# xdsopl/dwt

Hardware: AMD Instinct MI355X
Metric: Mpixels/s lossless encode+decode round-trip (higher is better)
Workload: dtype int32; 1 GPU; 4096x4096x1 8-bit synthetic smooth+noise frames, lossless, 128 frames per GPU per step (BASELINE.json configs[1] geometry); frames_per_gpu=128, parallelism=1 GPU

## Files before the change

dwt_amd/csrc/pack.hip:

```cpp
#include "hilbert_dev.h"

#include <stdlib.h>
#include <string.h>

namespace {

constexpr int TILE = 1024;
constexpr int NCUM = 32;
constexpr int MAX_PLANES = 16;
constexpr int MAX_SEGS = 3 * 16 * MAX_PLANES;
constexpr int SUB = 64;
constexpr int CHUNK = SUB * 64;
constexpr int GROUP = 64;

constexpr unsigned T_RUN = 0x0fffu, T_ESC = 0x0fffu, T_BREAK = 1u << 13, T_VOID = 1u << 14, T_NOSIGN = 1u << 15;

struct PackGeom {
	int levels, C, W, H;
	long total;
	const int *pyr;
	const short *fine16;
	unsigned lv16;
	unsigned sq_levels;
	int side[DWTX_MAX_LEVELS + 1];
	int pixels[DWTX_MAX_LEVELS + 1];
	int tile_first[DWTX_MAX_LEVELS + 1];
	const int *tile_base;
	const unsigned short *tile_cnt;
	const int *tile_blk;
};

struct ImgInfo {
	int planes[3];
	int pmax;
	int K;
	int E;
	unsigned T;
	int order0;
	unsigned hdr_bits;
	unsigned root_bits;
	unsigned meta_bits;
	unsigned cut;
	unsigned long long total_bits;
	unsigned long long nbytes;
	int error;
	int pad;
};

struct RunMap {
	unsigned keep, add;
};

struct Work {
	unsigned short *cum;
	unsigned *tile_mx;
	ImgInfo *info;
	int *seg_desc;
	int *seg_ebase;
	unsigned *seg_refs;
	unsigned long long *seg_rawoff;
	unsigned *brk_tok;
	int *segidx;
	unsigned *live;
	unsigned short *ent_ones, *ent_zeros, *ent_refs, *ent_tz;
	unsigned short *ent_seg;
	unsigned *ent_tokbase;
	unsigned *ent_refscum;
	unsigned *ent_refw;
	unsigned short *tok16;
	unsigned *tok_big;
	unsigned *stage;
	unsigned char *grp_ord;
	unsigned long long *lane_bits;
	unsigned char *sublut;
	unsigned char *lut;
	unsigned char *glut;
	unsigned char *chunk_entry;
	unsigned char *group_entry;
	unsigned long long *chunk_bits;
	unsigned long long *chunk_base;
	RunMap *carry_agg;
	unsigned *carry_in;
	unsigned *ent_blk;
	unsigned long long *stream_bits;
	int *slow;
	long ES, TS, NCS, NGS, NCB, SW;
	int NT, NTP;
	unsigned *seg_run;
};

__device__ __forceinline__ int lane_id()
{
	return __builtin_amdgcn_mbcnt_hi(~0u, __builtin_amdgcn_mbcnt_lo(~0u, 0));
}

__device__ __forceinline__ int popc_below(unsigned long long m)
{
	return __builtin_amdgcn_mbcnt_hi((unsigned)(m >> 32), __builtin_amdgcn_mbcnt_lo((unsigned)m, 0));
}

__device__ __forceinline__ int ilog2u(unsigned v) { return 31 - __builtin_clz(v); }

__device__ __forceinline__ void wave_sync()
{
	__builtin_amdgcn_fence(__ATOMIC_RELEASE, "wavefront");
	__builtin_amdgcn_wave_barrier();
	__builtin_amdgcn_fence(__ATOMIC_ACQUIRE, "wavefront");
}

__device__ __forceinline__ unsigned wave_incl_add(unsigned v)
{
	v += (unsigned)__builtin_amdgcn_update_dpp(0, (int)v, 0x111, 0xf, 0xf, false);
	v += (unsigned)__builtin_amdgcn_update_dpp(0, (int)v, 0x112, 0xf, 0xf, false);
	v += (unsigned)__builtin_amdgcn_update_dpp(0, (int)v, 0x114, 0xf, 0xf, false);
	v += (unsigned)__builtin_amdgcn_update_dpp(0, (int)v, 0x118, 0xf, 0xf, false);
	v += (unsigned)__builtin_amdgcn_update_dpp(0, (int)v, 0x142, 0xa, 0xf, false);
	v += (unsigned)__builtin_amdgcn_update_dpp(0, (int)v, 0x143, 0xc, 0xf, false);
	return v;
}

__device__ __forceinline__ unsigned bfm_mask(unsigned width)
{
	unsigned r;
	asm("v_bfm_b32 %0, %1, 0" : "=v"(r) : "v"(width));
	return r;
}
__device__ __forceinline__ int vli_top(int o, unsigned v) { return ilog2u(v + (1u << o)); }
__device__ __forceinline__ int vli_next(int top) { return top >= 2 ? top - 2 : 0; }

__device__ __forceinline__ void seg_unpack(int d, int &c, int &l, int &p)
{
	c = d & 15;
	l = (d >> 4) & 15;
	p = (d >> 8) - 1;
}

struct __attribute__((packed, aligned(4))) Int4U {
	int x, y, z, w;
};

__device__ __forceinline__ void load_tile16(const PackGeom &g, const int *__restrict__ lin, int plane, int l, int tile, int lane, int nvalid,
	int nv, unsigned *lds, int (&val)[16])
{
	if (((g.sq_levels >> l) & 1u) && nvalid == TILE) {
		if ((g.lv16 >> l) & 1u)
			load_square16(g.fine16 + (long)plane * g.total, g.W, g.side[l], g.tile_blk[tile], lane, lds, val);
		else
			load_square16(g.pyr + (long)plane * g.total, g.W, g.side[l], g.tile_blk[tile], lane, lds, val);
		return;
	}
	const int tbase = g.tile_base[tile];
	const int *src = lin + (long)plane * g.total + g.pixels[l] + tbase + 16 * lane;
	const int k = (int)(((uintptr_t)src >> 2) & 3);
// ... 481 lines not shown
	const unsigned tb = block_excl_scan(nt, wsum, tt);
	const unsigned rb = block_excl_scan(nr, wsum, rt);
	const unsigned wb = block_excl_scan((nr + 31u) >> 5, wsum, wt);
	if (e < E) {
		w.ent_tokbase[img * (w.ES + 1) + e] = tb;
		w.ent_refscum[img * (w.ES + 1) + e] = rb;
		w.ent_refw[img * (w.ES + 1) + e] = wb;
	}
	if (threadIdx.x == 0) {
		w.ent_blk[(img * w.NCB + blockIdx.x) * 3] = tt;
		w.ent_blk[(img * w.NCB + blockIdx.x) * 3 + 1] = rt;
		w.ent_blk[(img * w.NCB + blockIdx.x) * 3 + 2] = wt;
	}
}

__global__ __launch_bounds__(ENT_BLOCK) void k_entries_blocks(Work w)
{
	__shared__ unsigned wsum[16];
	const int img = blockIdx.x;
	ImgInfo &I = w.info[img];
	const int E = I.E;
	const int nb = (E + ENT_BLOCK - 1) / ENT_BLOCK;
	unsigned tok_run = 0, ref_run = 0, word_run = 0;
	for (int b0 = 0; b0 < nb; b0 += ENT_BLOCK) {
		const int b = b0 + threadIdx.x;
		unsigned *slot = w.ent_blk + (img * w.NCB + b) * 3;
		const unsigned t = b < nb ? slot[0] : 0u, r = b < nb ? slot[1] : 0u, wd = b < nb ? slot[2] : 0u;
		unsigned tt, rt, wt;
		const unsigned tb = block_excl_scan(t, wsum, tt);
		const unsigned rb = block_excl_scan(r, wsum, rt);
		const unsigned wb = block_excl_scan(wd, wsum, wt);
		if (b < nb) {
			slot[0] = tok_run + tb;
			slot[1] = ref_run + rb;
			slot[2] = word_run + wb;
		}
		tok_run += tt;
		ref_run += rt;
		word_run += wt;
	}
	if (threadIdx.x == 0) {
		w.ent_tokbase[img * (w.ES + 1) + E] = tok_run;
		w.ent_refscum[img * (w.ES + 1) + E] = ref_run;
		w.ent_refw[img * (w.ES + 1) + E] = word_run;
		I.T = tok_run + 1;
	}
}

__global__ __launch_bounds__(ENT_BLOCK) void k_entries_finish(Work w)
{
	const int img = blockIdx.y;
	const int e = blockIdx.x * ENT_BLOCK + threadIdx.x;
	if (e >= w.info[img].E)
		return;
	const unsigned *slot = w.ent_blk + (img * w.NCB + blockIdx.x) * 3;
	w.ent_tokbase[img * (w.ES + 1) + e] += slot[0];
	w.ent_refscum[img * (w.ES + 1) + e] += slot[1];
	w.ent_refw[img * (w.ES + 1) + e] += slot[2];
}

__global__ __launch_bounds__(ENT_BLOCK) void k_entries_segs(Work w)
{
	const int img = blockIdx.x;
	const int K = w.info[img].K;
	const int *eb = w.seg_ebase + (long)img * (MAX_SEGS + 1);
	const unsigned *tokbase = w.ent_tokbase + img * (w.ES + 1), *refscum = w.ent_refscum + img * (w.ES + 1);
	static_assert(MAX_SEGS <= ENT_BLOCK, "one thread per segment");
	const int k = threadIdx.x;
	if (k < K) {
		const unsigned refs = refscum[eb[k + 1]] - refscum[eb[k]];
		w.seg_refs[(long)img * MAX_SEGS + k] = refs;
		const int last = eb[k + 1] - 1;
		w.brk_tok[(long)img * MAX_SEGS + k] = tokbase[last] + w.ent_ones[img * w.ES + last];
	}
}

__global__ __launch_bounds__(ENT_BLOCK) void k_cut(Work w, long capacity, int cut_off)
{
	__shared__ unsigned long long need[MAX_SEGS];
	__shared__ int kc_sh;
	const int img = blockIdx.x;
	ImgInfo &I = w.info[img];
	const int K = I.K;
	const int *eb = w.seg_ebase + (long)img * (MAX_SEGS + 1);
	const unsigned *tokbase = w.ent_tokbase + img * (w.ES + 1);
	const int k = threadIdx.x;
	if (k < K) {
		const unsigned ones = tokbase[eb[k + 1]] - tokbase[eb[k]] - 1u;
		need[k] = 2ull * ones + w.seg_refs[(long)img * MAX_SEGS + k];
	}
	__syncthreads();
	if (threadIdx.x == 0) {
		int kc = K;
		if (capacity > 0 && !cut_off) {
			const unsigned long long limit = 8ull * ((unsigned long long)capacity + 1ull);
			unsigned long long at = I.hdr_bits;
			for (int j = 0; j < K; ++j) {
				if (at >= limit) {
					kc = j;
					break;
				}
				at += need[j];
			}
		}
		kc_sh = kc;
		I.cut = (unsigned)(K - kc);
		I.K = kc;
		I.E = eb[kc];
		I.T = tokbase[eb[kc]] + 1u;
	}
	__syncthreads();
	const int kc = kc_sh;
	if (threadIdx.x < 48) {
		const int *sx = w.segidx + ((long)img * 48 + threadIdx.x) * MAX_PLANES;
		unsigned m = 0;
		for (int p = 0; p < MAX_PLANES; ++p)
			m |= (sx[p] && sx[p] <= kc ? 1u : 0u) << p;
		w.live[(long)img * 48 + threadIdx.x] = m;
	}
}


__device__ __forceinline__ int tab8(int lane, int cls) { return cls * 128 + lane * 2; }
__device__ __forceinline__ int tab16(int lane, int cls) { return cls * 64 + lane; }
constexpr int ROWW = 34;
constexpr int ZS_DUMMY = TILE + 8 * MAX_PLANES, ZS_SLOTS = ZS_DUMMY + 8;

struct alignas(16) CodeLds {
	unsigned tab[1024];
	union {
		unsigned short zs[ZS_SLOTS];
		unsigned rows[(MAX_PLANES - 1) * ROWW];
	};
	unsigned short cum[MAX_PLANES + 2];
	unsigned short slot0[MAX_PLANES];
	unsigned gb[MAX_PLANES];
	unsigned long long rb[MAX_PLANES];
	int ent[MAX_PLANES];
};

template <int NQ>
struct Nib;
template <>
struct Nib<8> {
	typedef unsigned T;
	static constexpr T ONES = 0x11111111u, M0F = 0x0f0f0f0fu;
};
template <>
struct Nib<16> {
	typedef unsigned long long T;
	static constexpr T ONES = 0x1111111111111111ull, M0F = 0x0f0f0f0f0f0f0f0full;
};

__device__ __forceinline__ void transpose8(unsigned &lo, unsigned &hi)
{
	unsigned t;
	t = (lo ^ (lo >> 7)) & 0x00AA00AAu;
	lo ^= t ^ (t << 7);
	t = (hi ^ (hi >> 7)) & 0x00AA00AAu;
	hi ^= t ^ (t << 7);
	t = (lo ^ (lo >> 14)) & 0x0000CCCCu;
	lo ^= t ^ (t << 14);
	t = (hi ^ (hi >> 14)) & 0x0000CCCCu;
	hi ^= t ^ (t << 14);
	const unsigned nlo = (lo & 0x0F0F0F0Fu) | ((hi << 4) & 0xF0F0F0F0u);
	hi = ((lo >> 4) & 0x0F0F0F0Fu) | (hi & 0xF0F0F0F0u);
	lo = nlo;
}

__device__ __forceinline__ unsigned pext4_entry(unsigned i)
{
	const unsigned m = i >> 4, v = i & 15u;
	unsigned out = 0, k = 0;
#pragma unroll
	for (int j = 0; j < 4; ++j) {
		out |= (((v & m) >> j) & 1u) << k;
		k += (m >> j) & 1u;
	}
	return out;
}

typedef unsigned short ushort2_t __attribute__((ext_vector_type(2)));

__device__ __forceinline__ unsigned slots_to_tokens(unsigned a, unsigned before)
{
	const unsigned b = __builtin_amdgcn_alignbit(a, before, 16);
	const ushort2_t d = __builtin_bit_cast(ushort2_t, a & 0x03ff03ffu) - __builtin_bit_cast(ushort2_t, b & 0x03ff03ffu);
	return (a & 0x10001000u) | __builtin_bit_cast(unsigned, d);
}

template <int NQ, bool FULL>
__device__ __forceinline__ void code_tile(CodeLds &L, const unsigned char *pext4, const int (&val)[16], const Work &w, int img, int lane, int nvalid,
	int nv, int vb, int Pc, int tile_top, unsigned my_tokbase, int my_ent, unsigned long long my_rb)
{
	const int P = Pc < tile_top ? Pc : tile_top;
	typedef typename Nib<NQ>::T R_t;
	constexpr R_t ONES = Nib<NQ>::ONES, M0F = Nib<NQ>::M0F;
	constexpr int NB = NQ / 4;

	unsigned mag[16];
	unsigned sgn = 0;
	R_t Ra = 0, Rb = 0;
#pragma unroll
	for (int i = 0; i < 16; ++i) {
		const int v = val[i];
		const unsigned a = (unsigned)(v < 0 ? -v : v);
		mag[i] = a;
		sgn |= ((unsigned)v >> 31) << i;
		int t = 32 - __clz((int)a);
		t = t < NQ ? t : NQ;
		const int te = FULL || i < nv ? t : NQ;
		const R_t m = te < NQ ? ONES << (4 * te) : (R_t)0;
		if (i < 8)
			Ra += m;
		else
			Rb += m;
	}
	const R_t ev = (Ra & M0F) + (Rb & M0F);
	const R_t od = ((Ra >> 4) & M0F) + ((Rb >> 4) & M0F);
	unsigned E[NB], O[NB], cE[NB], cO[NB];
	const int nq = (P >> 2) + 1 < NB ? (P >> 2) + 1 : NB;
#pragma unroll
	for (int b = 0; b < NB; ++b) {
		const unsigned xe = (unsigned)(ev >> (16 * b)) & 0xffffu, xo = (unsigned)(od >> (16 * b)) & 0xffffu;
		const unsigned e0 = (xe & 0xffu) | ((xe & 0xff00u) << 8), o0 = (xo & 0xffu) | ((xo & 0xff00u) << 8);
		unsigned ei = 0, oi = 0;
		if (b < nq) {
			ei = wave_incl_add(e0);
			oi = wave_incl_add(o0);
		}
		cE[b] = (unsigned)__builtin_amdgcn_readlane((int)ei, 63);
		cO[b] = (unsigned)__builtin_amdgcn_readlane((int)oi, 63);
		E[b] = ei - e0;
		O[b] = oi - o0;
	}
#define ZL(q) ((((q) & 1 ? O[((q) >> 2) % NB] : E[((q) >> 2) % NB]) >> (16 * (((q) >> 1) & 1))) & 0xffffu)
#define CT(q) ((((q) & 1 ? cO[((q) >> 2) % NB] : cE[((q) >> 2) % NB]) >> (16 * (((q) >> 1) & 1))) & 0xffffu)
	unsigned first[NQ];
	{
		unsigned cur = 0;
#pragma unroll
		for (int p = NQ - 1; p >= 0; --p) {
			const unsigned c1 = p + 1 < P && p + 1 < NQ ? CT(p + 1) : (unsigned)nvalid, c0 = p < P ? CT(p) : (unsigned)nvalid;
			const unsigned tb = (unsigned)__builtin_amdgcn_readlane((int)my_tokbase, p);
			first[p] = cur + ((tb - cur) & 7u);
			cur = first[p] + (c1 - c0);
		}
	}
#pragma unroll
	for (int t = 1; t <= NQ; ++t) {
		if (t <= P) {
			const unsigned zlo = ZL(t - 1);
			const unsigned zhi = t < NQ && t < P ? ZL(t) : (unsigned)vb;
			if (NQ == 8)
				*reinterpret_cast<uint2 *>(&L.tab[tab8(lane, t - 1)]) = make_uint2(zlo, first[t - 1] + zhi - zlo);
			else
				L.tab[tab16(lane, t - 1)] = zlo | (zhi - zlo) << 10 | first[t - 1] << 20;
		}
	}
	if (lane == 0) {
#pragma unroll
		for (int q = 0; q <= MAX_PLANES; ++q)
			L.cum[q] = (unsigned short)(q < P && q < NQ ? CT(q) : (unsigned)nvalid);
#pragma unroll
		for (int q = 0; q < MAX_PLANES; ++q)
			L.slot0[q] = (unsigned short)(q < NQ ? first[q < NQ ? q : 0] : 0u);
	}
	wave_sync();

	if (lane < MAX_PLANES) {
		L.gb[lane] = my_ent >= 0 ? my_tokbase : ~0u;
		L.ent[lane] = my_ent;
		L.rb[lane] = my_rb;
	}
	wave_sync();

	auto cq = [&](int q) -> unsigned { return q < P && q < NQ ? CT(q) : (unsigned)nvalid; };

	wave_sync();
	for (int i = lane; i < (NQ - 1) * ROWW; i += 64)
		L.rows[i] = 0u;
	wave_sync();
	auto deposit = [&](int p, unsigned acc, unsigned cnt, unsigned zl, unsigned bit0) {
		const unsigned pos = (bit0 & 31u) + ((unsigned)vb - zl);
		if (cnt) {
			unsigned *row = L.rows + p * ROWW;
			const unsigned sh = pos & 31u;
			atomicOr(&row[pos >> 5], acc << sh);
			if (sh + cnt > 32u)
				atomicOr(&row[(pos >> 5) + 1], acc >> (32u - sh));
		}
	};
	unsigned *stage = w.stage + img * w.SW;
	auto row_out = [&](int p, int refs, unsigned long long bit0) {
		const int nw = (refs + 31) >> 5;
		if (lane < nw)
			stage[(bit0 >> 5) + lane] = L.rows[p * ROWW + lane];
	};
	if (NQ == 8) {
		unsigned A0 = mag[0] | mag[1] << 8 | mag[2] << 16 | mag[3] << 24, A1 = mag[4] | mag[5] << 8 | mag[6] << 16 | mag[7] << 24;
		unsigned B0 = mag[8] | mag[9] << 8 | mag[10] << 16 | mag[11] << 24, B1 = mag[12] | mag[13] << 8 | mag[14] << 16 | mag[15] << 24;
		transpose8(A0, A1);
		transpose8(B0, B1);
		const unsigned SA1 = (A1 >> 8) | (A1 >> 16) | (A1 >> 24), SB1 = (B1 >> 8) | (B1 >> 16) | (B1 >> 24);
		const unsigned SA0 = (A0 >> 8) | (A0 >> 16) | (A0 >> 24) | ((SA1 | A1) & 0xffu) * 0x01010101u;
		const unsigned SB0 = (B0 >> 8) | (B0 >> 16) | (B0 >> 24) | ((SB1 | B1) & 0xffu) * 0x01010101u;
		auto plane_string = [&](int p, unsigned Aw, unsigned SAw, unsigned Bw, unsigned SBw) {
			const int refs = nvalid - (int)L.cum[p + 1];
			if (refs <= 0 || L.ent[p] < 0)
				return;
			const unsigned sh8 = 8u * ((unsigned)p & 3u);
			const unsigned nA = (Aw >> sh8) & 0xffu, sA = (SAw >> sh8) & 0xffu, nB = (Bw >> sh8) & 0xffu, sB = (SBw >> sh8) & 0xffu;
			const unsigned e0 = pext4[((sA & 15u) << 4) | (nA & 15u)], e1 = pext4[(sA & 0xf0u) | (nA >> 4)];
			const unsigned e2 = pext4[((sB & 15u) << 4) | (nB & 15u)], e3 = pext4[(sB & 0xf0u) | (nB >> 4)];
			const unsigned c0 = (unsigned)__builtin_popcount(sA & 15u), c1 = (unsigned)__builtin_popcount(sA);
			const unsigned c2 = c1 + (unsigned)__builtin_popcount(sB & 15u), c3 = c1 + (unsigned)__builtin_popcount(sB);
			deposit(p, e0 | e1 << c0 | e2 << c1 | e3 << c2, c3, L.tab[tab8(lane, p + 1)] & 0x3ffu, (unsigned)L.rb[p]);
		};
		for (int p = P - 2; p >= 4; --p)
			plane_string(p, A1, SA1, B1, SB1);
		for (int p = P - 2 < 3 ? P - 2 : 3; p >= 0; --p)
			plane_string(p, A0, SA0, B0, SB0);
		wave_sync();
		for (int p = P - 2; p >= 0; --p) {
			const int refs = nvalid - (int)L.cum[p + 1];
			if (refs <= 0 || L.ent[p] < 0)
				continue;
			row_out(p, refs, L.rb[p]);
		}
	} else {
		for (int p = P - 2; p >= 0; --p) {
			const int refs = nvalid - (int)L.cum[p + 1];
			if (refs <= 0 || L.ent[p] < 0)
				continue;
			const unsigned thr = 2u << p;
			unsigned acc = 0, cnt = 0;
#pragma unroll
			for (int i = 0; i < 16; ++i) {
				const bool isref = mag[i] >= thr;
				acc |= (isref ? (mag[i] >> p) & 1u : 0u) << cnt;
				cnt += isref ? 1u : 0u;
			}
			deposit(p, acc, cnt, L.tab[tab16(lane, p + 1)] & 0x3ffu, (unsigned)L.rb[p]);
		}
		wave_sync();
		for (int p = P - 2; p >= 0; --p) {
			const int refs = nvalid - (int)L.cum[p + 1];
			if (refs <= 0 || L.ent[p] < 0)
				continue;
			row_out(p, refs, L.rb[p]);
		}
	}
	wave_sync();
	{
		R_t R = 0;
		constexpr int NB8 = NQ == 8 ? 8 : 2;
#pragma unroll
		for (int h = 0; h < 16 / NB8; ++h) {
			uint2 ent[NB8];
#pragma unroll
			for (int i = NB8 * h; i < NB8 * h + NB8; ++i) {
				const int t0 = min(32 - __clz((int)mag[i]), NQ);
				const int tm = t0 > 0 ? t0 - 1 : 0;
				if (NQ == 8) {
					ent[i % NB8] = *reinterpret_cast<const uint2 *>(&L.tab[tab8(lane, tm)]);
				} else {
					const unsigned e = L.tab[tab16(lane, tm)];
					ent[i % NB8] = make_uint2(e & 0x3ffu, (e >> 20) + ((e >> 10) & 0x3ffu));
				}
			}
#pragma unroll
			for (int i = NB8 * h; i < NB8 * h + NB8; ++i) {
				const int t = min(32 - __clz((int)mag[i]), NQ);
				const int tm = t > 0 ? t - 1 : 0;
				const unsigned x = (unsigned)(R >> (4 * tm));
				const unsigned lz_lo = x & 15u;
				const unsigned lz_hi = t < NQ ? (x >> 4) & 15u : (unsigned)i;
				const unsigned slot = mag[i] ? ent[i % NB8].y + lz_hi - lz_lo : (unsigned)(ZS_DUMMY + (lane & 7));
				L.zs[slot] = (unsigned short)(ent[i % NB8].x + lz_lo + ((sgn >> i) & 1u) * 0x1000u);
				const int te = FULL || i < nv ? t : NQ;
				R += te < NQ ? ONES << (4 * te) : (R_t)0;
			}
		}
	}
	wave_sync();
	{
		unsigned first_tok = 0;
		int first_slot = -1;
		if (lane < MAX_PLANES) {
			const int p = lane;
			const unsigned c0 = L.cum[p], c1 = L.cum[p + 1];
			const unsigned ones = c1 - c0, slot0 = L.slot0[p];
			if (ones) {
				first_slot = (int)slot0;
				first_tok = L.zs[slot0];
			}
			if (my_ent >= 0)
				w.ent_tz[img * w.ES + my_ent] = (unsigned short)(ones ? c0 - (L.zs[slot0 + ones - 1] & 0x3ffu) : c0);
		}
		const int nslots = (int)(first[0] + (cq(1) - cq(0)));
		uint4 *zq = reinterpret_cast<uint4 *>(L.zs);
		const int nblk = (nslots + 511) >> 9;
		unsigned before[3];
#pragma unroll
		for (int k = 0; k < 3; ++k)
			before[k] = k < nblk && 512 * k + 8 * lane > 0 && 512 * k + 8 * lane <= ZS_DUMMY ? (unsigned)L.zs[512 * k + 8 * lane - 1] << 16 : 0u;
		wave_sync();
#pragma unroll
		for (int k = 0; k < 3; ++k)
			if (k < nblk && 64 * k + lane < ZS_DUMMY / 8) {
				const uint4 a = zq[64 * k + lane];
				zq[64 * k + lane] = make_uint4(slots_to_tokens(a.x, before[k]), slots_to_tokens(a.y, a.x), slots_to_tokens(a.z, a.y), slots_to_tokens(a.w, a.z));
			}
		wave_sync();
		if (first_slot >= 0)
			L.zs[first_slot] = (unsigned short)first_tok;
		wave_sync();
		unsigned short *tok16 = w.tok16 + img * w.TS;
		auto plane_out = [&](unsigned tb, unsigned slot0, int ones) {
			unsigned short *dst = tok16 + tb;
			const unsigned short *src = L.zs + slot0;
			const int head = min(ones, (int)((8u - (tb & 7u)) & 7u));
			const int chunks = (ones - head) >> 3, tail0 = head + 8 * chunks;
			const int e = lane < 8 ? lane : tail0 + lane - 8;
			if (lane < 8 ? lane < head : (lane < 16 && e < ones))
				dst[e] = src[e];
			for (int c = lane; c < chunks; c += 64)
				*reinterpret_cast<uint4 *>(dst + head + 8 * c) = *reinterpret_cast<const uint4 *>(src + head + 8 * c);
		};
		for (int p = P > 0 ? P - 1 : 0; p >= 0; --p) {
			const unsigned c0 = (unsigned)__builtin_amdgcn_readfirstlane((int)L.cum[p]), c1 = (unsigned)__builtin_amdgcn_readfirstlane((int)L.cum[p + 1]);
			const int ones = (int)(c1 - c0);
			const unsigned gb = (unsigned)__builtin_amdgcn_readfirstlane((int)L.gb[p]);
			if (ones <= 0 || gb == ~0u)
				continue;
			plane_out(gb, (unsigned)__builtin_amdgcn_readfirstlane((int)L.slot0[p]), ones);
		}
	}

#undef ZL
#undef CT
}

template <bool WIDE>
__device__ __forceinline__ void code_one(const PackGeom &g, const int *__restrict__ lin, const Work &w, CodeLds &L, const unsigned char *pext4, int tile,
	int plane, int lane)
{
	const int img = plane / g.C, c = plane - img * g.C;
	const ImgInfo &I = w.info[img];
	{
	int l = 0;
	while (l + 1 < g.levels && tile >= g.tile_first[l + 1])
		++l;
	const int j = tile - g.tile_first[l];
	const int nvalid = g.tile_cnt[tile];
	const int P = I.planes[c] < MAX_PLANES ? I.planes[c] : MAX_PLANES;
	const unsigned live = w.live[(long)img * 48 + c * 16 + l];
	if (!live)
		return;
	const unsigned tile_or = w.tile_mx[(long)plane * w.NTP + tile];
	const int tile_top = tile_or ? ilog2u(tile_or) + 1 : 0;
	if (!(live & ((1u << (tile_top < 31 ? tile_top : 31)) - 1u))) {
		if (lane < MAX_PLANES && ((live >> lane) & 1u)) {
			const int k = w.segidx[((long)img * 48 + c * 16 + l) * MAX_PLANES + lane] - 1;
			w.ent_tz[img * w.ES + w.seg_ebase[(long)img * (MAX_SEGS + 1) + k] + j] = (unsigned short)nvalid;
		}
		return;
	}
	const int first = 16 * lane;
	const int nv = nvalid - first < 0 ? 0 : nvalid - first > 16 ? 16 : nvalid - first;
	const int vb = first < nvalid ? first : nvalid;

	static_assert(sizeof(L.tab) >= sizeof(unsigned) * SQ_WORDS, "the class table doubles as the square's staging area");
	int val[16];
	load_tile16(g, lin, plane, l, tile, lane, nvalid, nv, L.tab, val);
// ... 442 lines not shown
		const unsigned xs[2] = { x2.x, x2.y };
#pragma unroll
		for (int h = 0; h < 2; ++h) {
			const unsigned x = xs[h];
			if (pair_is_special(x)) {
				const unsigned v[2] = { token_run(x & 0xffffu, big, tb + 4 * q + 2 * h), token_run(x >> 16, big, tb + 4 * q + 2 * h + 1) };
				pair_bits(x, v, tb + 4 * q + 2 * h, lo, count_raw, btok, srefs, K, tokbits, rawbits);
			} else {
				pair_bits_plain(x, tb + 4 * q + 2 * h, lo, count_raw, btok, srefs, K, tokbits, rawbits);
			}
		}
	}
	if (met)
		hi = lo;
	return qmet;
}

__device__ __forceinline__ void walk_bits(const unsigned *my, const unsigned *big, long tb, int o, int qend, bool count_raw,
	const unsigned *btok, const unsigned *srefs, int K, unsigned &tokbits, unsigned long long &rawbits)
{
#pragma unroll 2
	for (int q = 0; q < qend; ++q) {
		const uint2 x2 = *reinterpret_cast<const uint2 *>(my + 2 * q);
		const unsigned xs[2] = { x2.x, x2.y };
#pragma unroll
		for (int h = 0; h < 2; ++h) {
			const unsigned x = xs[h];
			if (pair_is_special(x)) {
				const unsigned v[2] = { token_run(x & 0xffffu, big, tb + 4 * q + 2 * h), token_run(x >> 16, big, tb + 4 * q + 2 * h + 1) };
				pair_bits(x, v, tb + 4 * q + 2 * h, o, count_raw, btok, srefs, K, tokbits, rawbits);
			} else {
				pair_bits_plain(x, tb + 4 * q + 2 * h, o, count_raw, btok, srefs, K, tokbits, rawbits);
			}
		}
	}
}

constexpr int FSUBS = 63;

struct WalkLds {
	unsigned tok[64 * WROW];
};

constexpr int GO_WAVES = 2;

__global__ __launch_bounds__(64 * GO_WAVES) void k_gorder(Work w)
{
	__shared__ WalkLds lds[GO_WAVES];
	const int lane = threadIdx.x & 63, wv = threadIdx.x >> 6;
	const long wave = (long)blockIdx.x * GO_WAVES + wv;
	const int img = blockIdx.y;
	const ImgInfo &I = w.info[img];
	const long T = I.T;
	const long nsub = (T + SUB - 1) / SUB;
	if (wave * FSUBS >= nsub)
		return;
	const unsigned short *tok16 = w.tok16 + img * w.TS;
	const unsigned *big = w.tok_big + img * w.TS;
	unsigned *rows = lds[wv].tok;
	const long S = wave * FSUBS - 1 + lane;
	const long tfirst = (wave * FSUBS - 1) * SUB;
	stage_tokens(rows, tok16, tfirst, T, lane);
	wave_sync();
	const unsigned *my = rows + lane * WROW;
	const long tb = S * SUB;
	int lo = 0, hi = 31;
	const bool valid = S >= 0 && S < nsub;
	const bool produces = lane >= 1 && valid;
	const unsigned *btok = w.brk_tok + (long)img * MAX_SEGS, *srefs = w.seg_refs + (long)img * MAX_SEGS;
	unsigned tokbits;
	unsigned long long rawbits;
	const int qmet = walk_order2(my, big, tb, lo, hi, produces, btok, srefs, I.K, tokbits, rawbits);
	int exitv = lo;
	bool exit_known = lo == hi || !valid;
	int o = 0;
	bool entry_known = false;
	for (int it = 0; it < 4; ++it) {
		o = __shfl_up(exitv, 1);
		entry_known = __shfl_up((int)exit_known, 1) != 0 && lane >= 1;
		if (S == 0) {
			o = I.order0;
			entry_known = true;
		}
		const bool resolve = valid && !exit_known && entry_known;
		if (!ballot64(resolve))
			break;
		const int e = walk_order(my, big, tb, o);
		if (resolve) {
			exitv = e;
			exit_known = true;
		}
	}
	if (ballot64(lane >= 1 && valid && !entry_known)) {
		if (lane == 0)
			atomicOr(w.slow + img, 1);
		return;
	}
	walk_bits(my, big, tb, o, qmet, produces, btok, srefs, I.K, tokbits, rawbits);
	unsigned long long total;
	const unsigned long long pre = wave_excl_scan64(produces ? tokbits + rawbits : 0ull, total);
	if (produces) {
		w.lane_bits[img * w.NCS * 64 + S] = pre;
		w.grp_ord[img * w.NCS * 64 + S] = (unsigned char)o;
	}
	if (lane == 0)
		w.chunk_bits[img * w.NCS + wave] = total;
}


__device__ __forceinline__ void lut_body(const Work &w, long vbx, int img)
{
	const int lane = threadIdx.x & 63, half = lane >> 5, s = lane & 31;
	const long chunk = (vbx * 4 + (threadIdx.x >> 6)) * 2 + half;
	const unsigned T = w.info[img].T;
	const long nchunks = ((long)T + CHUNK - 1) / CHUNK;
	const long chunk_a = chunk - half;
	if (chunk_a >= nchunks)
		return;
	const bool live = chunk < nchunks;
	const unsigned short *tok16 = w.tok16 + img * w.TS;
	const unsigned *big = w.tok_big + img * w.TS;
	unsigned char *sub = w.sublut + (img * w.NCS + chunk) * 64 * 32;
	auto one = [&](long t) -> unsigned {
		if (t >= (long)T)
			return 0x80000000u;
		const unsigned tk = tok16[t];
		return token_run(tk, big, t) | ((tk & T_VOID) ? 0x80000000u : 0u);
	};
	auto fetch = [&](int q, unsigned &ra, unsigned &rb) {
		const long ta = chunk_a * CHUNK + q * SUB + lane;
		ra = one(ta);
		rb = one(ta + CHUNK);
	};
	int o = s;
	unsigned na, nb;
	fetch(0, na, nb);
	for (int q = 0; q < 64; ++q) {
		if (live)
			sub[q * 32 + s] = (unsigned char)o;
		const unsigned ra = na, rb = nb;
		if (q + 1 < 64)
			fetch(q + 1, na, nb);
#pragma unroll
		for (int t = 0; t < 64; ++t) {
			const unsigned a = __builtin_amdgcn_readlane(ra, t), b = __builtin_amdgcn_readlane(rb, t);
			const unsigned v = half ? b : a;
			o = vli_step(o, v & 0x7fffffffu, v >> 31);
		}
	}
	if (live)
		w.lut[(img * w.NCS + chunk) * 32 + s] = (unsigned char)o;
}

__global__ __launch_bounds__(256) void k_lut(Work w)
{
	const int img = blockIdx.y;
	if (!w.slow[img])
		return;
	const long nvb = (w.NCS + 7) / 8;
	for (long vb = blockIdx.x; vb < nvb; vb += gridDim.x)
		lut_body(w, vb, img);
}

__device__ __forceinline__ void chain_groups_body(const Work &w, long vbx, int img)
{
	const int lane = threadIdx.x & 63, half = lane >> 5, s = lane & 31;
	const long group = (vbx * 4 + (threadIdx.x >> 6)) * 2 + half;
	const unsigned T = w.info[img].T;
	const long nchunks = ((long)T + CHUNK - 1) / CHUNK;
	const long ngroups = (nchunks + GROUP - 1) / GROUP;
	if (group >= ngroups)
		return;
	const unsigned char *lut = w.lut + img * w.NCS * 32;
	int o = s;
	for (long c = group * GROUP; c < min((group + 1) * GROUP, nchunks); ++c)
		o = lut[c * 32 + o];
	w.glut[(img * w.NGS + group) * 32 + s] = (unsigned char)o;
}

__global__ __launch_bounds__(256) void k_chain_groups(Work w)
{
	const int img = blockIdx.y;
	if (!w.slow[img])
		return;
	const long nvb = (w.NGS + 7) / 8;
	for (long vb = blockIdx.x; vb < nvb; vb += gridDim.x)
		chain_groups_body(w, vb, img);
}

__global__ __launch_bounds__(1024) void k_chain_image(Work w)
{
	const int img = blockIdx.x;
	if (!w.slow[img])
		return;
	const ImgInfo &I = w.info[img];
	const long nchunks = ((long)I.T + CHUNK - 1) / CHUNK;
	const long ngroups = (nchunks + GROUP - 1) / GROUP;
	unsigned char *gentry = w.group_entry + img * w.NGS;
	if (threadIdx.x == 0) {
		int o = I.order0;
		for (long gq = 0; gq < ngroups; ++gq) {
			gentry[gq] = (unsigned char)o;
			o = w.glut[(img * w.NGS + gq) * 32 + o];
		}
	}
	__syncthreads();
	__threadfence_block();
	const unsigned char *lut = w.lut + img * w.NCS * 32;
	unsigned char *centry = w.chunk_entry + img * w.NCS;
	for (long gq = threadIdx.x; gq < ngroups; gq += 1024) {
		int o = gentry[gq];
		for (long c = gq * GROUP; c < min((gq + 1) * GROUP, nchunks); ++c) {
			centry[c] = (unsigned char)o;
			o = lut[c * 32 + o];
		}
	}
}

__device__ __forceinline__ void gorder_exact_body(const Work &w, unsigned *rows, long chunk, int img)
{
	const int lane = threadIdx.x & 63;
	const ImgInfo &I = w.info[img];
	const long T = I.T;
	const long nchunks = (T + CHUNK - 1) / CHUNK;
	if (chunk >= nchunks)
		return;
	const unsigned short *tok16 = w.tok16 + img * w.TS;
	const unsigned *big = w.tok_big + img * w.TS;
	wave_sync();
	stage_tokens(rows, tok16, chunk * CHUNK, T, lane);
	wave_sync();
	const long S = chunk * 64 + lane;
	const int o = w.sublut[((img * w.NCS + chunk) * 64 + lane) * 32 + w.chunk_entry[img * w.NCS + chunk]];
	const bool produces = S * SUB < T;
	unsigned tokbits = 0;
	unsigned long long rawbits = 0;
	walk_bits(rows + lane * WROW, big, S * SUB, o, 16, produces, w.brk_tok + (long)img * MAX_SEGS, w.seg_refs + (long)img * MAX_SEGS, I.K,
		tokbits, rawbits);
	unsigned long long total;
	const unsigned long long pre = wave_excl_scan64(produces ? tokbits + rawbits : 0ull, total);
	if (produces) {
		w.lane_bits[img * w.NCS * 64 + S] = pre;
		w.grp_ord[img * w.NCS * 64 + S] = (unsigned char)o;
	}
	if (lane == 0)
		w.chunk_bits[img * w.NCS + chunk] = total;
}

__global__ __launch_bounds__(256) void k_gorder_exact(Work w)
{
	__shared__ WalkLds lds[4];
	const int img = blockIdx.y;
	if (!w.slow[img])
		return;
	const long nvb = (w.NCS + 3) / 4;
	for (long vb = blockIdx.x; vb < nvb; vb += gridDim.x)
		gorder_exact_body(w, lds[threadIdx.x >> 6].tok, vb * 4 + (threadIdx.x >> 6), img);
}

constexpr int EWIN = 768;

struct EmitLds {
	unsigned tok[64 * HROW];
	unsigned win[EWIN];
};

__global__ __launch_bounds__(256) __attribute__((amdgpu_waves_per_eu(5))) void k_emit(Work w, unsigned *out, long out_words)
{
	__shared__ EmitLds lds[4];
	const int lane = threadIdx.x & 63, wv = threadIdx.x >> 6;
	const long wave = (long)blockIdx.x * 4 + wv;
	const int img = blockIdx.y;
	const ImgInfo &I = w.info[img];
	const long T = I.T;
	const long ngroups = (T + SUB - 1) / SUB;
	if (wave * 64 >= ngroups)
		return;
	const unsigned short *tok16 = w.tok16 + img * w.TS;
	const unsigned *big = w.tok_big + img * w.TS;
	const unsigned *srefs = w.seg_refs + (long)img * MAX_SEGS;
	const unsigned *btok = w.brk_tok + (long)img * MAX_SEGS;
	unsigned *rows = lds[wv].tok, *win = lds[wv].win;
	for (int i = lane; i < EWIN; i += 64)
		win[i] = 0u;
	const long S = wave * 64 + lane;
	const bool live = S < ngroups;
	const int per = w.slow[img] ? 64 : FSUBS;
	unsigned long long pos = 0;
	int o = 0;
	if (live) {
		pos = w.chunk_base[img * w.NCS + S / per] + w.lane_bits[img * w.NCS * 64 + S];
		o = w.grp_ord[img * w.NCS * 64 + S];
	}
	const long wbase = (long)(__shfl(pos, 0) >> 5);
	unsigned *dst = out + img * out_words;
	wave_sync();
	auto put_word = [&](long wi, unsigned v) {
		if (!v)
			return;
		const unsigned long rel = (unsigned long)(wi - wbase);
		if (rel < (unsigned long)EWIN)
			__hip_atomic_fetch_or((__attribute__((address_space(3))) unsigned *)win + rel, v, __ATOMIC_RELAXED, __HIP_MEMORY_SCOPE_WORKGROUP);
		else if (wi < out_words)
			atomicOr(dst + wi, v);
	};
	long widx = (long)(pos >> 5);
// ... 447 lines not shown
		return DWTX_ERR_ARG;
	DWTX_ENTER(ctx);
	DWTX_CHECK_DIMS(W, H);
	PackGeom g;
	Work w;
	dwtx_tiles tiles;
	const int rc = pack_geometry(ctx, W, H, C, n, g, w, tiles);
	if (rc)
		return rc;
	hipLaunchKernelGGL(k_hist_init, dim3(dwtx_cdiv(w.NT * (NCUM / 2), 256), n * C), dim3(256), 0, ctx->stream, g, w);
	DWTX_LAUNCH_CHECK();
	sink->cum32 = reinterpret_cast<unsigned *>(w.cum);
	sink->tile_mx = w.tile_mx;
	sink->NT = w.NT;
	sink->NTP = w.NTP;
	sink->tiles = tiles;
	return DWTX_OK;
}

#ifdef DWTX_DEBUG_HOOKS
extern "C" int dwtx_debug_hist_copy(dwtx_ctx *ctx, int W, int H, int C, int n, unsigned *host_cum32, unsigned *host_mx, int *NT, int *NTP, int *tile_first)
{
	PackGeom g;
	Work w;
	dwtx_tiles tiles;
	const int rc = pack_geometry(ctx, W, H, C, n, g, w, tiles);
	if (rc)
		return rc;
	*NT = w.NT;
	*NTP = w.NTP;
	for (int l = 0; l <= g.levels; ++l)
		tile_first[l] = tiles.tile_first[l];
	if (host_cum32) {
		DWTX_HIP(hipMemcpyAsync(host_cum32, w.cum, sizeof(unsigned) * 16 * (size_t)n * C * w.NT, hipMemcpyDeviceToHost, ctx->stream));
		DWTX_HIP(hipMemcpyAsync(host_mx, w.tile_mx, sizeof(unsigned) * (size_t)n * C * w.NTP, hipMemcpyDeviceToHost, ctx->stream));
		DWTX_HIP(hipStreamSynchronize(ctx->stream));
	}
	return DWTX_OK;
}
#endif

int dwtx_encode_planes_ex(dwtx_ctx *ctx, const int32_t *lin, const int32_t *pyr, unsigned sq_levels, unsigned hist_levels, int W, int H, int C,
	int n, long capacity, uint8_t *out, size_t out_stride, dwtx_stream_info *dev_info, dwtx_p16 p16, dwtx_index *dev_index)
{
	if (!ctx || !lin || !out || !dev_info || (C != 1 && C != 3) || n < 1 || n > 65535 || (out_stride & 3) || out_stride < 8)
		return DWTX_ERR_ARG;
	DWTX_ENTER(ctx);
	DWTX_CHECK_DIMS(W, H);
	if (sq_levels && (!pyr || (sq_levels & ~dwtx_square_levels(W, H)) || ((uintptr_t)pyr & 15)))
		return DWTX_ERR_ARG;
	PackGeom g;
	Work w;
	dwtx_tiles tiles;
	{
		const int rc = pack_geometry(ctx, W, H, C, n, g, w, tiles);
		if (rc)
			return rc;
	}
	g.pyr = pyr;
	g.sq_levels = sq_levels;
	g.fine16 = p16.planes;
	g.lv16 = p16.planes ? p16.levels : 0u;
	if (p16.planes && ((p16.levels & ~sq_levels) || ((uintptr_t)p16.planes & 15)))
		return DWTX_ERR_ARG;
	const int NT = tiles.NT;
	int hist_tiles = NT;
	for (int l = g.levels - 1; l >= 0 && ((hist_levels >> l) & 1u); --l)
		hist_tiles = tiles.tile_first[l];
	w.ES = (long)NT * C * MAX_PLANES + 16;
	w.TS = ((long)C * (g.total - g.pixels[0]) + MAX_SEGS + 8 + 63) / 64 * 64;
	w.NCS = (w.TS / SUB + FSUBS - 1) / FSUBS + 2;
	w.NGS = (w.NCS + GROUP - 1) / GROUP;
	w.NCB = (w.ES + CARRY_BLOCK - 1) / CARRY_BLOCK;
	w.SW = (long)(((unsigned long long)C * (unsigned long long)(g.total - g.pixels[0]) * (MAX_PLANES - 1) + 31) / 32) + w.ES + 64;
	const int nplanes = n * C;

	const size_t imgs = n;
	char *small = carve(ctx, SLOT_PK_SMALL, [&](Carve &c) {
		c.take(w.info, imgs);
		c.take(w.slow, imgs);
		c.take(w.stream_bits, imgs);
		c.take(w.seg_desc, imgs * MAX_SEGS);
		c.take(w.seg_ebase, imgs * (MAX_SEGS + 1));
		c.take(w.seg_refs, imgs * MAX_SEGS);
		c.take(w.seg_rawoff, imgs * MAX_SEGS);
		c.take(w.brk_tok, imgs * MAX_SEGS);
		c.take(w.segidx, imgs * 48 * MAX_PLANES);
		c.take(w.live, imgs * 48);
		c.take(w.seg_run, imgs * MAX_SEGS);
	});
	if (!small)
		return DWTX_ERR_NOMEM;
	DWTX_HIP(hipMemsetAsync(w.info, 0, (char *)w.seg_desc - (char *)w.info, ctx->stream));
	if (ctx->opt[DWTX_OPT_EXACT_ORDERS])
		DWTX_HIP(hipMemsetD32Async((hipDeviceptr_t)w.slow, 1, (size_t)n, ctx->stream));

	char *ent = carve(ctx, SLOT_PK_ENT, [&](Carve &c) {
		c.take(w.ent_ones, imgs * w.ES);
		c.take(w.ent_zeros, imgs * w.ES);
		c.take(w.ent_refs, imgs * w.ES);
		c.take(w.ent_tz, imgs * w.ES);
		c.take(w.ent_seg, imgs * w.ES);
		c.take(w.ent_tokbase, imgs * (w.ES + 1));
		c.take(w.ent_refscum, imgs * (w.ES + 1));
		c.take(w.ent_refw, imgs * (w.ES + 1));
		c.take(w.carry_agg, imgs * w.NCB);
		c.take(w.carry_in, imgs * w.NCB);
		c.take(w.ent_blk, imgs * w.NCB * 3);
	});
	if (!ent)
		return DWTX_ERR_NOMEM;

	w.tok_big = (unsigned *)dwtx_scratch(ctx, SLOT_PK_TOKBIG, sizeof(unsigned) * (size_t)n * w.TS);
	w.tok16 = (unsigned short *)dwtx_scratch(ctx, SLOT_PK_TOK16, sizeof(unsigned short) * (size_t)n * w.TS);
	w.stage = (unsigned *)dwtx_scratch(ctx, SLOT_PK_STAGE, sizeof(unsigned) * (size_t)n * w.SW);
	if (!w.tok_big || !w.tok16 || !w.stage)
		return DWTX_ERR_NOMEM;

	w.sublut = (unsigned char *)dwtx_scratch(ctx, SLOT_PK_LUT, (size_t)n * w.NCS * 64 * 32);
	char *ch = carve(ctx, SLOT_PK_CHUNK, [&](Carve &c) {
		c.take(w.lut, imgs * w.NCS * 32);
		c.take(w.glut, imgs * w.NGS * 32);
		c.take(w.chunk_entry, imgs * w.NCS);
		c.take(w.group_entry, imgs * w.NGS);
		c.take(w.grp_ord, imgs * w.NCS * 64);
		c.take(w.chunk_bits, imgs * w.NCS);
		c.take(w.chunk_base, imgs * w.NCS);
		c.take(w.lane_bits, imgs * w.NCS * 64);
	});
	if (!w.sublut || !ch)
		return DWTX_ERR_NOMEM;

	hipStream_t s = ctx->stream;
	const long out_words = (long)(out_stride / 4);
	unsigned *outw = (unsigned *)out;

	if (hist_tiles > 0)
		hipLaunchKernelGGL(k_hist, dim3(dwtx_cdiv(hist_tiles, 4 * HIST_TPW), nplanes), dim3(256), 0, s, g, lin, w, hist_levels);
	hipLaunchKernelGGL(k_plan, dim3(n), dim3(1024), 0, s, g, lin, w, outw, out_words, capacity);
	hipLaunchKernelGGL(k_entries_count, dim3((unsigned)w.NCB, n), dim3(ENT_BLOCK), 0, s, g, w);
	hipLaunchKernelGGL(k_entries_blocks, dim3(n), dim3(ENT_BLOCK), 0, s, w);
	hipLaunchKernelGGL(k_entries_finish, dim3((unsigned)w.NCB, n), dim3(ENT_BLOCK), 0, s, w);
	hipLaunchKernelGGL(k_entries_segs, dim3(n), dim3(ENT_BLOCK), 0, s, w);
	hipLaunchKernelGGL(k_cut, dim3(n), dim3(ENT_BLOCK), 0, s, w, capacity, (int)(ctx->opt[DWTX_OPT_NO_CAPACITY_CUT] != 0));
	hipLaunchKernelGGL(k_code<false>, dim3(dwtx_cdiv(NT, 4), nplanes), dim3(256), 0, s, g, lin, w);
	hipLaunchKernelGGL(k_code<true>, dim3(dwtx_cdiv(NT, 4) < 64 ? dwtx_cdiv(NT, 4) : 64, nplanes), dim3(256), 0, s, g, lin, w);
	hipLaunchKernelGGL(k_carry_local, dim3((unsigned)w.NCB, n), dim3(CARRY_THREADS), 0, s, w);
	hipLaunchKernelGGL(k_carry_blocks, dim3(n), dim3(CARRY_BLOCK), 0, s, w);
	if (dev_index)
		hipLaunchKernelGGL(k_carry_apply<true>, dim3((unsigned)w.NCB, n), dim3(CARRY_THREADS), 0, s, w);
	else
		hipLaunchKernelGGL(k_carry_apply<false>, dim3((unsigned)w.NCB, n), dim3(CARRY_THREADS), 0, s, w);
	hipLaunchKernelGGL(k_gorder, dim3((int)((w.NCS + GO_WAVES - 1) / GO_WAVES), n), dim3(64 * GO_WAVES), 0, s, w);
	hipLaunchKernelGGL(k_lut, dim3(512, n), dim3(256), 0, s, w);
	hipLaunchKernelGGL(k_chain_groups, dim3(64, n), dim3(256), 0, s, w);
	hipLaunchKernelGGL(k_chain_image, dim3(n), dim3(1024), 0, s, w);
	hipLaunchKernelGGL(k_gorder_exact, dim3(512, n), dim3(256), 0, s, w);
	hipLaunchKernelGGL(k_bitscan, dim3(n), dim3(1024), 0, s, w, capacity);
	{
		const long cb = (out_words / 4 + 256) / 256;
		hipLaunchKernelGGL(k_clear_stream, dim3((unsigned)(cb < 1024 ? cb : 1024), n), dim3(256), 0, s, w, outw, out_words);
	}
	hipLaunchKernelGGL(k_emit, dim3((unsigned)((w.TS / CHUNK + 1 + 3) / 4), n), dim3(256), 0, s, w, outw, out_words);
	hipLaunchKernelGGL(k_refcopy, dim3(256, n), dim3(256), 0, s, w, outw, out_words);
	if (dev_index)
		hipLaunchKernelGGL(k_index, dim3(n), dim3(IDX_THREADS), 0, s, g, w, dev_index);
	DWTX_LAUNCH_CHECK();
	static_assert(sizeof(dwtx_stream_info) == sizeof(ImgInfo), "ImgInfo is the device image of dwtx_stream_info");
	DWTX_HIP(hipMemcpyAsync(dev_info, w.info, sizeof(ImgInfo) * (size_t)n, hipMemcpyDeviceToDevice, s));
	return DWTX_OK;
}
```

Baseline: 87290 Mpixels/s.

## Derive NQ=8 plane counts from transposed bit planes; size exact-order grids to work

For 8-plane tiles, per-plane zero-prefix counts are now computed with nibble popcounts over the already-needed transposed bit-plane words. This replaces the per-value clz and one-hot accumulation, and the transpose is shared with plane-string emission. Lane 0's serial writes of cum/slot0 become one write per lane, and row clearing is bounded by the actual plane count P instead of NQ. The k_lut, k_chain_groups and k_gorder_exact grids are capped at the needed block count (at most 64) rather than fixed 512/64. The count semantics for partial tiles (nv) must match the old clz path exactly, which carries correctness risk.

```diff
diff --git a/dwt_amd/csrc/pack.hip b/dwt_amd/csrc/pack.hip
--- a/dwt_amd/csrc/pack.hip
+++ b/dwt_amd/csrc/pack.hip
@@ -1,4 +1,5 @@
 #include "hilbert_dev.h"
+#include "plane_counts.h"
 
 #include <stdlib.h>
 #include <string.h>
@@ -786,22 +787,6 @@
 	static constexpr T ONES = 0x1111111111111111ull, M0F = 0x0f0f0f0f0f0f0f0full;
 };
 
-__device__ __forceinline__ void transpose8(unsigned &lo, unsigned &hi)
-{
-	unsigned t;
-	t = (lo ^ (lo >> 7)) & 0x00AA00AAu;
-	lo ^= t ^ (t << 7);
-	t = (hi ^ (hi >> 7)) & 0x00AA00AAu;
-	hi ^= t ^ (t << 7);
-	t = (lo ^ (lo >> 14)) & 0x0000CCCCu;
-	lo ^= t ^ (t << 14);
-	t = (hi ^ (hi >> 14)) & 0x0000CCCCu;
-	hi ^= t ^ (t << 14);
-	const unsigned nlo = (lo & 0x0F0F0F0Fu) | ((hi << 4) & 0xF0F0F0F0u);
-	hi = ((lo >> 4) & 0x0F0F0F0Fu) | (hi & 0xF0F0F0F0u);
-	lo = nlo;
-}
-
 __device__ __forceinline__ unsigned pext4_entry(unsigned i)
 {
 	const unsigned m = i >> 4, v = i & 15u;
@@ -834,39 +819,58 @@
 
 	unsigned mag[16];
 	unsigned sgn = 0;
-	R_t Ra = 0, Rb = 0;
 #pragma unroll
 	for (int i = 0; i < 16; ++i) {
 		const int v = val[i];
-		const unsigned a = (unsigned)(v < 0 ? -v : v);
-		mag[i] = a;
+		mag[i] = (unsigned)(v < 0 ? -v : v);
 		sgn |= ((unsigned)v >> 31) << i;
-		int t = 32 - __clz((int)a);
-		t = t < NQ ? t : NQ;
-		const int te = FULL || i < nv ? t : NQ;
-		const R_t m = te < NQ ? ONES << (4 * te) : (R_t)0;
-		if (i < 8)
-			Ra += m;
-		else
-			Rb += m;
-	}
-	const R_t ev = (Ra & M0F) + (Rb & M0F);
-	const R_t od = ((Ra >> 4) & M0F) + ((Rb >> 4) & M0F);
+	}
+	unsigned e0[NB], o0[NB];
+	LanePlanes8 pl;
+	if constexpr (NQ == 8) {
+		lane_planes8(mag, pl);
+		unsigned c[2];
+		lane_counts8(pl, FULL ? 16u : (unsigned)nv, c[0], c[1]);
+#pragma unroll
+		for (int b = 0; b < NB; ++b) {
+			e0[b] = counts_even(c[b]);
+			o0[b] = counts_odd(c[b]);
+		}
+	} else {
+		R_t Ra = 0, Rb = 0;
+#pragma unroll
+		for (int i = 0; i < 16; ++i) {
+			int t = 32 - __clz((int)mag[i]);
+			t = t < NQ ? t : NQ;
+			const int te = FULL || i < nv ? t : NQ;
+			const R_t m = te < NQ ? ONES << (4 * te) : (R_t)0;
+			if (i < 8)
+				Ra += m;
+			else
+				Rb += m;
+		}
+		const R_t ev = (Ra & M0F) + (Rb & M0F);
+		const R_t od = ((Ra >> 4) & M0F) + ((Rb >> 4) & M0F);
+#pragma unroll
+		for (int b = 0; b < NB; ++b) {
+			const unsigned xe = (unsigned)(ev >> (16 * b)) & 0xffffu, xo = (unsigned)(od >> (16 * b)) & 0xffffu;
+			e0[b] = (xe & 0xffu) | ((xe & 0xff00u) << 8);
+			o0[b] = (xo & 0xffu) | ((xo & 0xff00u) << 8);
+		}
+	}
 	unsigned E[NB], O[NB], cE[NB], cO[NB];
 	const int nq = (P >> 2) + 1 < NB ? (P >> 2) + 1 : NB;
 #pragma unroll
 	for (int b = 0; b < NB; ++b) {
-		const unsigned xe = (unsigned)(ev >> (16 * b)) & 0xffffu, xo = (unsigned)(od >> (16 * b)) & 0xffffu;
-		const unsigned e0 = (xe & 0xffu) | ((xe & 0xff00u) << 8), o0 = (xo & 0xffu) | ((xo & 0xff00u) << 8);
 		unsigned ei = 0, oi = 0;
 		if (b < nq) {
-			ei = wave_incl_add(e0);
-			oi = wave_incl_add(o0);
+			ei = wave_incl_add(e0[b]);
+			oi = wave_incl_add(o0[b]);
 		}
 		cE[b] = (unsigned)__builtin_amdgcn_readlane((int)ei, 63);
 		cO[b] = (unsigned)__builtin_amdgcn_readlane((int)oi, 63);
-		E[b] = ei - e0;
-		O[b] = oi - o0;
+		E[b] = ei - e0[b];
+		O[b] = oi - o0[b];
 	}
 #define ZL(q) ((((q) & 1 ? O[((q) >> 2) % NB] : E[((q) >> 2) % NB]) >> (16 * (((q) >> 1) & 1))) & 0xffffu)
 #define CT(q) ((((q) & 1 ? cO[((q) >> 2) % NB] : cE[((q) >> 2) % NB]) >> (16 * (((q) >> 1) & 1))) & 0xffffu)
@@ -892,13 +896,21 @@
 				L.tab[tab16(lane, t - 1)] = zlo | (zhi - zlo) << 10 | first[t - 1] << 20;
 		}
 	}
-	if (lane == 0) {
-#pragma unroll
-		for (int q = 0; q <= MAX_PLANES; ++q)
-			L.cum[q] = (unsigned short)(q < P && q < NQ ? CT(q) : (unsigned)nvalid);
-#pragma unroll
-		for (int q = 0; q < MAX_PLANES; ++q)
-			L.slot0[q] = (unsigned short)(q < NQ ? first[q < NQ ? q : 0] : 0u);
+	if (lane <= MAX_PLANES) {
+		const int q = lane;
+		unsigned tot = 0;
+#pragma unroll
+		for (int b = 0; b < NB; ++b)
+			tot = (q >> 2) == b ? (q & 1 ? cO[b] : cE[b]) : tot;
+		const unsigned ct = (tot >> (16 * ((q >> 1) & 1))) & 0xffffu;
+		L.cum[q] = (unsigned short)(q < P && q < NQ ? ct : (unsigned)nvalid);
+		if (q < MAX_PLANES) {
+			unsigned f = 0;
+#pragma unroll
+			for (int p = 0; p < NQ; ++p)
+				f = q == p ? first[p] : f;
+			L.slot0[q] = (unsigned short)f;
+		}
 	}
 	wave_sync();
 
@@ -912,7 +924,7 @@
 	auto cq = [&](int q) -> unsigned { return q < P && q < NQ ? CT(q) : (unsigned)nvalid; };
 
 	wave_sync();
-	for (int i = lane; i < (NQ - 1) * ROWW; i += 64)
+	for (int i = lane; i < (P - 1) * ROWW; i += 64)
 		L.rows[i] = 0u;
 	wave_sync();
 	auto deposit = [&](int p, unsigned acc, unsigned cnt, unsigned zl, unsigned bit0) {
@@ -932,13 +944,6 @@
 			stage[(bit0 >> 5) + lane] = L.rows[p * ROWW + lane];
 	};
 	if (NQ == 8) {
-		unsigned A0 = mag[0] | mag[1] << 8 | mag[2] << 16 | mag[3] << 24, A1 = mag[4] | mag[5] << 8 | mag[6] << 16 | mag[7] << 24;
-		unsigned B0 = mag[8] | mag[9] << 8 | mag[10] << 16 | mag[11] << 24, B1 = mag[12] | mag[13] << 8 | mag[14] << 16 | mag[15] << 24;
-		transpose8(A0, A1);
-		transpose8(B0, B1);
-		const unsigned SA1 = (A1 >> 8) | (A1 >> 16) | (A1 >> 24), SB1 = (B1 >> 8) | (B1 >> 16) | (B1 >> 24);
-		const unsigned SA0 = (A0 >> 8) | (A0 >> 16) | (A0 >> 24) | ((SA1 | A1) & 0xffu) * 0x01010101u;
-		const unsigned SB0 = (B0 >> 8) | (B0 >> 16) | (B0 >> 24) | ((SB1 | B1) & 0xffu) * 0x01010101u;
 		auto plane_string = [&](int p, unsigned Aw, unsigned SAw, unsigned Bw, unsigned SBw) {
 			const int refs = nvalid - (int)L.cum[p + 1];
 			if (refs <= 0 || L.ent[p] < 0)
@@ -952,9 +957,9 @@
 			deposit(p, e0 | e1 << c0 | e2 << c1 | e3 << c2, c3, L.tab[tab8(lane, p + 1)] & 0x3ffu, (unsigned)L.rb[p]);
 		};
 		for (int p = P - 2; p >= 4; --p)
-			plane_string(p, A1, SA1, B1, SB1);
+			plane_string(p, pl.A1, pl.SA1, pl.B1, pl.SB1);
 		for (int p = P - 2 < 3 ? P - 2 : 3; p >= 0; --p)
-			plane_string(p, A0, SA0, B0, SB0);
+			plane_string(p, pl.A0, pl.SA0, pl.B0, pl.SB0);
 		wave_sync();
 		for (int p = P - 2; p >= 0; --p) {
 			const int refs = nvalid - (int)L.cum[p + 1];
@@ -1703,6 +1708,7 @@
 		w.lut[(img * w.NCS + chunk) * 32 + s] = (unsigned char)o;
 }
 
+constexpr int EXACT_GRID = 64;
 __global__ __launch_bounds__(256) void k_lut(Work w)
 {
 	const int img = blockIdx.y;
@@ -2456,10 +2462,13 @@
 	else
 		hipLaunchKernelGGL(k_carry_apply<false>, dim3((unsigned)w.NCB, n), dim3(CARRY_THREADS), 0, s, w);
 	hipLaunchKernelGGL(k_gorder, dim3((int)((w.NCS + GO_WAVES - 1) / GO_WAVES), n), dim3(64 * GO_WAVES), 0, s, w);
-	hipLaunchKernelGGL(k_lut, dim3(512, n), dim3(256), 0, s, w);
-	hipLaunchKernelGGL(k_chain_groups, dim3(64, n), dim3(256), 0, s, w);
-	hipLaunchKernelGGL(k_chain_image, dim3(n), dim3(1024), 0, s, w);
-	hipLaunchKernelGGL(k_gorder_exact, dim3(512, n), dim3(256), 0, s, w);
+	{
+		auto grid = [](long nvb) { return (unsigned)(nvb < 1 ? 1 : nvb < EXACT_GRID ? nvb : EXACT_GRID); };
+		hipLaunchKernelGGL(k_lut, dim3(grid((w.NCS + 7) / 8), n), dim3(256), 0, s, w);
+		hipLaunchKernelGGL(k_chain_groups, dim3(grid((w.NGS + 7) / 8), n), dim3(256), 0, s, w);
+		hipLaunchKernelGGL(k_chain_image, dim3(n), dim3(1024), 0, s, w);
+		hipLaunchKernelGGL(k_gorder_exact, dim3(grid((w.NCS + 3) / 4), n), dim3(256), 0, s, w);
+	}
 	hipLaunchKernelGGL(k_bitscan, dim3(n), dim3(1024), 0, s, w, capacity);
 	{
 		const long cb = (out_words / 4 + 256) / 256;
diff --git a/dwt_amd/csrc/plane_counts.h b/dwt_amd/csrc/plane_counts.h
--- /dev/null
+++ b/dwt_amd/csrc/plane_counts.h
@@ -0,0 +1,74 @@
+#ifndef DWTX_PLANE_COUNTS_H
+#define DWTX_PLANE_COUNTS_H
+
+#if defined(__HIPCC__)
+#define DWTX_HD __host__ __device__
+#else
+#define DWTX_HD
+#endif
+
+DWTX_HD inline void transpose8(unsigned &lo, unsigned &hi)
+{
+	unsigned t;
+	t = (lo ^ (lo >> 7)) & 0x00AA00AAu;
+	lo ^= t ^ (t << 7);
+	t = (hi ^ (hi >> 7)) & 0x00AA00AAu;
+	hi ^= t ^ (t << 7);
+	t = (lo ^ (lo >> 14)) & 0x0000CCCCu;
+	lo ^= t ^ (t << 14);
+	t = (hi ^ (hi >> 14)) & 0x0000CCCCu;
+	hi ^= t ^ (t << 14);
+	const unsigned nlo = (lo & 0x0F0F0F0Fu) | ((hi << 4) & 0xF0F0F0F0u);
+	hi = ((lo >> 4) & 0x0F0F0F0Fu) | (hi & 0xF0F0F0F0u);
+	lo = nlo;
+}
+
+struct LanePlanes8 {
+	unsigned A0, A1, B0, B1, SA0, SA1, SB0, SB1;
+};
+
+DWTX_HD inline void lane_planes8(const unsigned (&mag)[16], LanePlanes8 &pl)
+{
+	unsigned A0 = mag[0] | mag[1] << 8 | mag[2] << 16 | mag[3] << 24, A1 = mag[4] | mag[5] << 8 | mag[6] << 16 | mag[7] << 24;
+	unsigned B0 = mag[8] | mag[9] << 8 | mag[10] << 16 | mag[11] << 24, B1 = mag[12] | mag[13] << 8 | mag[14] << 16 | mag[15] << 24;
+	transpose8(A0, A1);
+	transpose8(B0, B1);
+	pl.SA1 = (A1 >> 8) | (A1 >> 16) | (A1 >> 24);
+	pl.SB1 = (B1 >> 8) | (B1 >> 16) | (B1 >> 24);
+	pl.SA0 = (A0 >> 8) | (A0 >> 16) | (A0 >> 24) | ((pl.SA1 | A1) & 0xffu) * 0x01010101u;
+	pl.SB0 = (B0 >> 8) | (B0 >> 16) | (B0 >> 24) | ((pl.SB1 | B1) & 0xffu) * 0x01010101u;
+	pl.A0 = A0;
+	pl.A1 = A1;
+	pl.B0 = B0;
+	pl.B1 = B1;
+}
+
+DWTX_HD inline unsigned popc_nibbles(unsigned x)
+{
+	x -= (x >> 1) & 0x55555555u;
+	return (x & 0x33333333u) + ((x >> 2) & 0x33333333u);
+}
+
+DWTX_HD inline unsigned counts_le4(unsigned ua, unsigned ub, unsigned nv)
+{
+	const unsigned s = popc_nibbles(ua) + popc_nibbles(ub);
+	const unsigned above = (s & 0x0f0f0f0fu) + ((s >> 4) & 0x0f0f0f0fu);
+	return nv * 0x01010101u - above;
+}
+
+DWTX_HD inline void lane_counts8(const LanePlanes8 &pl, unsigned nv, unsigned &lo, unsigned &hi)
+{
+	lo = counts_le4(pl.SA0 | pl.A0, pl.SB0 | pl.B0, nv);
+	hi = counts_le4(pl.SA1 | pl.A1, pl.SB1 | pl.B1, nv);
+}
+
+DWTX_HD inline unsigned counts_even(unsigned c) { return c & 0x00ff00ffu; }
+DWTX_HD inline unsigned counts_odd(unsigned c) { return (c >> 8) & 0x00ff00ffu; }
+
+DWTX_HD inline unsigned counts_ev(unsigned lo, unsigned hi)
+{
+	return (lo & 0xffu) | ((lo >> 8) & 0xff00u) | ((hi & 0xffu) << 16) | ((hi & 0xff0000u) << 8);
+}
+DWTX_HD inline unsigned counts_od(unsigned lo, unsigned hi) { return counts_ev(lo >> 8, hi >> 8); }
+
+#endif
```

Measured after the change: 88080 Mpixels/s (median of 6 runs). Within noise of the previous version (+0.9%).
